# chrischoy/DeepGlobalRegistration

Measured on AMD Instinct MI355X. Metric: pair registrations/sec (FCGF x2 + 1-NN + 6-D inlier net + gate + weighted Procrustes + SE(3) refinement), higher is better.
Workload: dtype f32 results via 2 x f16 split operands (3 f16 MFMA products per MAC, f32 accumulate); k = 1 convs, kNN re-evaluation and registration in exact f32, SVD in f64

## Files before the change

deepglobalregistration_amd/_lib.py:

```python
import ctypes as C
import os
import threading

import torch

_HERE = os.path.dirname(os.path.abspath(__file__))
LIB_PATH = os.environ.get('DGR_HIP_LIB') or os.path.join(_HERE, 'lib', 'libdgr_hip.so')

DGR_OK, DGR_EINVAL, DGR_EHIP, DGR_ENOMEM, DGR_ESVD, DGR_EINTERNAL = 0, -1, -2, -3, -4, -5
STATUS_OK, STATUS_LOW_CONFIDENCE, STATUS_SVD_FAILED, STATUS_SAFEGUARD = 0, 1, 2, 3
STATUS_FLAG_ICP_SKIPPED, STATUS_MASK = 0x100, 0xff

c_i32p, c_i64p, c_f32p, c_f64p = (C.POINTER(C.c_int32), C.POINTER(C.c_int64),
                                  C.POINTER(C.c_float), C.POINTER(C.c_double))
vp = C.c_void_p


class WeightDesc(C.Structure):
    _fields_ = [('name', C.c_char_p), ('data', vp), ('numel', C.c_int64)]


class Params(C.Structure):
    _fields_ = [('clip_weight_thresh', C.c_float), ('voxel_size', C.c_float),
                ('inlier_feature_type', C.c_int), ('max_iter', C.c_int),
                ('max_break_count', C.c_int), ('break_threshold_ratio', C.c_double),
                ('skip_refinement', C.c_int), ('safeguard', C.c_int), ('ransac_hypotheses', C.c_int64),
                ('ransac_seed', C.c_uint32), ('use_icp', C.c_int)]


class PgParams(C.Structure):
    _fields_ = [('mu', C.c_double), ('reference_node', C.c_int), ('max_iter', C.c_int), ('rel_tol', C.c_double)]


SIGNATURES = {
    'dgr_last_error': (C.c_char_p, []),
    'dgr_version': (C.c_char_p, []),
    'dgr_ctx_create': (C.c_int, [C.c_int, C.POINTER(vp)]),
    'dgr_ctx_destroy': (None, [vp]),
    'dgr_ctx_workspace_bytes': (C.c_int64, [vp]),
    'dgr_ctx_create_partition_stream': (C.c_int, [vp, C.c_int, C.c_int, C.POINTER(vp)]),
    'dgr_voxelize': (C.c_int, [vp, vp, C.c_int, C.c_int64, C.c_double, C.c_int32, vp, vp, vp, c_i64p, vp]),
    'dgr_net_create': (C.c_int, [vp, C.c_int, C.c_int, C.c_int, C.c_int, C.c_int,
                                 C.POINTER(WeightDesc), C.c_int, C.POINTER(vp)]),
    'dgr_net_create_device': (C.c_int, [vp, C.c_int, C.c_int, C.c_int, C.c_int, C.c_int,
                                        C.POINTER(WeightDesc), C.c_int, C.POINTER(vp)]),
    'dgr_net_destroy': (None, [vp]),
    'dgr_net_param_bytes': (C.c_int64, [vp]),
    'dgr_net_share': (C.c_int, [vp, vp, C.POINTER(vp)]),
    'dgr_net_sharers': (C.c_int, [vp]),
    'dgr_net_set_wide_coarse': (C.c_int, [vp, C.c_int]),
    'dgr_resunet_forward': (C.c_int, [vp, vp, vp, vp, C.c_int64, vp, vp]),
    'dgr_net_get_intermediate': (C.c_int, [vp, vp, C.c_char_p, vp, C.c_int64, c_i64p, c_i64p]),
    'dgr_net_get_tensor': (C.c_int, [vp, vp, C.c_char_p, C.c_int, vp, C.c_int64, c_i64p, c_i64p]),
    'dgr_net_layer_stats': (C.c_int, [vp, vp, C.c_int, c_i64p]),
    'dgr_net_num_layers': (C.c_int, [vp]),
    'dgr_net_rerun_layer': (C.c_int, [vp, vp, C.c_int, C.c_int, c_f32p, c_f32p]),
    'dgr_maps_create': (C.c_int, [vp, vp, C.c_int64, C.c_int, C.c_int, C.POINTER(vp), vp]),
    'dgr_maps_destroy': (None, [vp]),
    'dgr_maps_get_coords': (C.c_int, [vp, C.c_int, vp, C.c_int64, c_i64p]),
    'dgr_maps_get_kernel_map': (C.c_int, [vp, C.c_int, C.c_int, vp, C.c_int64, vp, vp, C.c_int64,
                                          c_i64p, c_i64p]),
    'dgr_maps_create_ex': (C.c_int, [vp, vp, C.c_int64, C.c_int, C.c_int, C.c_int, C.POINTER(vp), vp]),
    'dgr_maps_get_raw': (C.c_int, [vp, C.c_char_p, C.c_int, C.c_char_p, vp, C.c_int64, c_i64p, c_i64p]),
# ... 142 lines not shown
```

deepglobalregistration_amd/csrc/ctx.hip:

```cpp
#include <stdarg.h>
#include <time.h>
#include <string.h>

#include "dgr_internal.h"

static thread_local char g_err[1024] = "";

void dgr_set_error(const char *fmt, ...) {
  va_list ap;
  va_start(ap, fmt);
  vsnprintf(g_err, sizeof(g_err), fmt, ap);
  va_end(ap);
}

extern "C" const char *dgr_last_error(void) { return g_err; }
extern "C" const char *dgr_version(void) { return "dgr_hip 0.4 (gfx950)"; }

static constexpr size_t kAlign = 256;
static constexpr size_t kMinChunk = (size_t)256 << 20;

bool dgr_workspace_fill(uint32_t *word) {
  static const char *env = getenv("DGR_WORKSPACE_FILL");
  static const uint32_t w = env ? (uint32_t)strtoul(env, nullptr, 16) : 0u;
  if (word) *word = w;
  return env != nullptr;
// ... 89 lines not shown
  }
  return ev[used++];
}

void DgrEventPool::release() {
  for (auto e : ev) (void)hipEventDestroy(e);
  ev.clear();
  used = 0;
}

extern "C" int dgr_ctx_create(int device, dgr_ctx **out) {
  DGR_REQUIRE(out != nullptr, "dgr_ctx_create: out is NULL");
  int count = 0;
  DGR_HIP_CHECK(hipGetDeviceCount(&count));
  DGR_REQUIRE(device >= 0 && device < count, "dgr_ctx_create: device %d out of range (%d visible)",
              device, count);
  DGR_HIP_CHECK(hipSetDevice(device));
  hipDeviceProp_t prop;
  DGR_HIP_CHECK(hipGetDeviceProperties(&prop, device));
  dgr_ctx *ctx = new dgr_ctx();
  ctx->device = device;
  ctx->num_cus = prop.multiProcessorCount > 0 ? prop.multiProcessorCount : 256;
  ctx->all_cus = ctx->num_cus;
  *out = ctx;
  return DGR_OK;
}

extern "C" int dgr_ctx_create_partition_stream(dgr_ctx *ctx, int part, int nparts, dgr_stream *out) {
  DGR_REQUIRE(ctx != nullptr && out != nullptr, "dgr_ctx_create_partition_stream: NULL argument");
  DGR_REQUIRE(nparts == 1 || nparts == 2 || nparts == 4, "partition stream: nparts = %d (1, 2 or 4)", nparts);
  DGR_REQUIRE(part >= 0 && part < nparts, "partition stream: part %d of %d", part, nparts);
  DGR_HIP_CHECK(hipSetDevice(ctx->device));
  *out = nullptr;
  if (ctx->part_stream) {
    DGR_HIP_CHECK(hipDeviceSynchronize());
    DGR_HIP_CHECK(hipStreamDestroy(ctx->part_stream));
    ctx->part_stream = nullptr;
    ctx->num_cus = ctx->all_cus;
  }
  if (nparts == 1) return DGR_OK;
  const int n = ctx->all_cus, xcds = 8;
  DGR_REQUIRE(n % (xcds * 8) == 0, "partition stream: %d compute units are not 8 XCDs x 8 k slots", n);
  const int words = (n + 31) / 32;
  std::vector<uint32_t> mask(words, 0u);
  int mine = 0;
  for (int b = 0; b < n; ++b)
// ... 14 lines not shown
    ctx->pin_bytes = 0;
    const size_t want = bytes < 4096 ? 4096 : bytes * 2;
    DGR_HIP_CHECK(hipHostMalloc((void **)&ctx->pin, want, hipHostMallocDefault));
    ctx->pin_bytes = want;
  }
  *out = ctx->pin;
  return DGR_OK;
}

int dgr_ctx_wait(dgr_ctx *ctx, hipStream_t stream, long predicted_ns) {
  static const bool spin = getenv("DGR_SPIN_SYNC") != nullptr;
  if (spin) {
    DGR_HIP_CHECK(hipStreamSynchronize(stream));
    return DGR_OK;
  }
  if (!ctx->wait_ev) DGR_HIP_CHECK(hipEventCreateWithFlags(&ctx->wait_ev, hipEventDisableTiming));
  DGR_HIP_CHECK(hipEventRecord(ctx->wait_ev, stream));
  struct timespec t0, t1;
  clock_gettime(CLOCK_MONOTONIC, &t0);
  auto elapsed_ns = [&]() -> long {
    clock_gettime(CLOCK_MONOTONIC, &t1);
    return (t1.tv_sec - t0.tv_sec) * 1000000000l + (t1.tv_nsec - t0.tv_nsec);
  };
  if (predicted_ns > 300000) {
    const long ns = predicted_ns / 5 * 4;
    struct timespec first = {ns / 1000000000l, ns % 1000000000l};
    nanosleep(&first, nullptr);
  }
  for (;;) {
    const hipError_t e = hipEventQuery(ctx->wait_ev);
    if (e == hipSuccess) break;
    if (e != hipErrorNotReady) DGR_HIP_CHECK(e);
    const long el = elapsed_ns();
    if (predicted_ns > 300000 && el < predicted_ns + predicted_ns / 10) {
      if (predicted_ns > 8000000) {
        struct timespec nap = {0, 30000};
        nanosleep(&nap, nullptr);
      }
      continue;
    }
    long ns = el / 64;
    struct timespec nap = {0, ns < 10000 ? 10000 : ns > 200000 ? 200000 : ns};
    nanosleep(&nap, nullptr);
  }
  ctx->last_wait_ns = elapsed_ns();
  return DGR_OK;
}

extern "C" void dgr_ctx_destroy(dgr_ctx *ctx) {
  if (!ctx) return;
  (void)hipSetDevice(ctx->device);
  (void)hipDeviceSynchronize();
  if (ctx->wait_ev) (void)hipEventDestroy(ctx->wait_ev);
  if (ctx->pin) (void)hipHostFree(ctx->pin);
  if (ctx->part_stream) (void)hipStreamDestroy(ctx->part_stream);
  ctx->arena.release();
  ctx->events.release();
  delete ctx;
}

extern "C" int64_t dgr_ctx_workspace_bytes(dgr_ctx *ctx) {
  return ctx ? (int64_t)ctx->arena.reserved() : 0;
}

extern "C" int dgr_debug_workspace_peek(dgr_ctx *ctx, int64_t nwords, uint32_t *host_out) {
  DGR_REQUIRE(ctx != nullptr && host_out != nullptr && nwords > 0, "dgr_debug_workspace_peek: bad argument");
  DGR_HIP_CHECK(hipSetDevice(ctx->device));
  DGR_HIP_CHECK(hipDeviceSynchronize());
  DGR_CHECK(ctx->arena.reset());
  uint32_t *p;
  DGR_ALLOC(p, ctx->arena, uint32_t, nwords);
// ... 80 lines not shown
```

deepglobalregistration_amd/csrc/dgr_internal.h:

```cpp
#pragma once
#include <hip/hip_runtime.h>
#include <stdint.h>
#include <stdio.h>
#include <stdlib.h>
#include <string>
#include <vector>

#include "../../include/dgr_hip.h"

void dgr_set_error(const char *fmt, ...);

#define DGR_HIP_CHECK(expr)                                                                  \
  do {                                                                                       \
    hipError_t _e = (expr);                                                                  \
    if (_e != hipSuccess) {                                                                  \
      dgr_set_error("%s:%d: %s failed: %s", __FILE__, __LINE__, #expr, hipGetErrorString(_e)); \
      return DGR_EHIP;                                                                       \
    }                                                                                        \
  } while (0)

#define DGR_CHECK(expr)          \
  do {                           \
    int _r = (expr);             \
    if (_r != DGR_OK) return _r; \
  } while (0)

#define DGR_REQUIRE(cond, ...)     \
  do {                             \
    if (!(cond)) {                 \
// ... 185 lines not shown
int dgr_conv_dense_launch(const DgrConvOsLaunch &a, hipStream_t stream, const char **kernel_name = nullptr);
bool dgr_conv_up_supported(int cin, int cin_pad, int cout);
int dgr_conv_up_launch(const DgrConvOsLaunch &a, hipStream_t stream, const char **kernel_name = nullptr);
int dgr_l2_normalize_rows(const float *in, int in_ld, float *out, int out_ld, int c, int relu,
                          const int32_t *n_dev, int64_t n_cap, hipStream_t stream);

struct DgrBatchOutputs {
  const void *ptr[5] = {nullptr, nullptr, nullptr, nullptr, nullptr};
  int64_t numel[5] = {0, 0, 0, 0, 0};
  uint64_t generation = 0;
};

struct DgrEventPool {
  std::vector<hipEvent_t> ev;
  size_t used = 0;
  hipEvent_t next();
  void release();
};

constexpr int DGR_KNN_TRACE_FIELDS = 8;

struct dgr_ctx {
  int device = 0;
  int num_cus = 256;
  DgrArena arena;
  bool profiling = false;
  float stage_ms[9] = {0, 0, 0, 0, 0, 0, 0, 0, 0};
  int64_t conv_launches = 0;
  DgrBatchOutputs last;
  std::vector<double> last_T64;
  DgrEventPool events;
  std::vector<std::pair<hipEvent_t, hipEvent_t>> conv_spans, gemm_spans, map3_spans, map6_spans;
  std::vector<float> conv_span_ms, gemm_span_ms;
  std::vector<unsigned long long *> conv_clks;
  std::vector<float> conv_clk_us;
  std::vector<const char *> conv_kinds;
  int32_t *flag_dev = nullptr;
  hipEvent_t wait_ev = nullptr;
  long last_wait_ns = 0;
  double batch_ns_per_row = 0;
  double pairs_ns_per_row = 0;
  unsigned char *pin = nullptr;
  size_t pin_bytes = 0;
  hipStream_t part_stream = nullptr;
  int all_cus = 256;
  bool knn_trace = false;
  std::vector<int32_t> knn_trace_rows;
  std::vector<int64_t> knn_trace_q0;
};

int dgr_ctx_pinned(dgr_ctx *ctx, size_t bytes, unsigned char **out);
int dgr_flag_error(int32_t flag);

int dgr_ctx_wait(dgr_ctx *ctx, hipStream_t stream, long predicted_ns = 0);

int dgr_resunet_forward_impl(dgr_ctx *ctx, dgr_net *net, const int32_t *coords, const float *feats,
                             int64_t N, float *out, hipStream_t stream);
int dgr_ctx_collect_profile(dgr_ctx *ctx);
void dgr_ctx_begin_profile(dgr_ctx *ctx);

int dgr_knn1_batch_impl(dgr_ctx *ctx, const float *F0, const int64_t *off0, const float *F1, const int64_t *off1,
                        int npairs, int C, int squared, int64_t *idx_out, float *dist_out, hipStream_t stream);
int dgr_knn1_impl(dgr_ctx *ctx, const float *F0, int64_t N0, const float *F1, int64_t N1, int C,
                  int squared, int64_t *idx_out, float *dist_out, hipStream_t stream);
int dgr_inlier_inputs_impl(const int32_t *coords0, const float *xyz0, int64_t N0,
                           const int32_t *coords1, const float *xyz1, const int64_t *idx1,
                           int feature_type, int32_t *coords6, float *feats, hipStream_t stream);
int dgr_icp_impl(dgr_ctx *ctx, const float *src, int64_t N0, const float *dst, int64_t N1, double max_dist,
                 const double *T_init, int max_iter, double rel_fitness, double rel_rmse, double *T_out,
                 double *stats_out, hipStream_t stream);
int dgr_ransac_impl(dgr_ctx *ctx, const float *X, const float *Y, int64_t N, double max_dist, int64_t num_hypotheses,
                    uint32_t seed, double *T_out, double *stats_out, hipStream_t stream);
// ... 44 lines not shown
```

deepglobalregistration_amd/csrc/net.hip:

```cpp
#include <math.h>
#include <stdlib.h>
#include <string.h>

#include <algorithm>
#include <memory>
#include <string>

#include "dgr_internal.h"

constexpr int CH[5] = {0, 32, 64, 128, 256};
constexpr int TR[5] = {0, 64, 64, 64, 128};
static constexpr float BN_EPS = 1e-5f;

enum Tn : int { NO = -1, X, T1, Y1, CAT1, S1T, S1, T2, Y2, CAT2, S2T, S2, T4, Y4, CAT4, S4T, S4, T8, Y8, S8,
                U4, V4, U2, V2, U1, V1, H, OUT, N_TENSORS };
constexpr int W_CIN = -1, W_COUT = -2;
struct TensorRow { const char *name; int lvl; Tn buf; int col0, cols, relu; };
static const TensorRow TENSORS[N_TENSORS] = {
    {"X", 0, X, 0, W_CIN, 0},
    {"T1", 0, T1, 0, CH[1], 0}, {"Y1", 0, Y1, 0, CH[1], 1},
    {"CAT1", 0, CAT1, 0, TR[2] + CH[1], 1}, {"S1T", 0, CAT1, 0, TR[2], 1}, {"S1", 0, CAT1, TR[2], CH[1], 1},
    {"T2", 1, T2, 0, CH[2], 0}, {"Y2", 1, Y2, 0, CH[2], 1},
    {"CAT2", 1, CAT2, 0, TR[3] + CH[2], 1}, {"S2T", 1, CAT2, 0, TR[3], 1}, {"S2", 1, CAT2, TR[3], CH[2], 1},
    {"T4", 2, T4, 0, CH[3], 0}, {"Y4", 2, Y4, 0, CH[3], 1},
// ... 737 lines not shown
      const LayerRow &row = LAYERS[li];
      const DgrLayer &L = net->W->layers[li];
      maps[li] = map_of(ms, row.map, TENSORS[row.in].lvl, TENSORS[row.out].lvl);
      kinds[li] = layer_kind(ms, f.wide3, L, maps[li], row.res != NO, ms.cm[TENSORS[row.in].lvl].n_cap,
                             net->width(TENSORS[row.in].buf));
      if (rule_major(kinds[li])) need = std::max(need, maps[li].km->pair_cap * L.cout);
    }
    DGR_ALLOC(f.ybuf, A, float, need);
  }
  Tensor t[N_TENSORS];
  const bool fuse_l2 = net->normalize && net->cout <= 32;
  for (int i = 0; i < N_TENSORS; ++i) {
    const TensorRow &row = TENSORS[i];
    t[i].ld = net->width(row.buf);
    t[i].relu = row.relu;
    if (row.buf != i) t[i].ptr = t[row.buf].ptr + row.col0;
    else if (i == X) t[i].ptr = const_cast<float *>(feats);
    else if (i == OUT && (!net->normalize || fuse_l2)) t[i].ptr = out;
    else t[i].ptr = A.get<float>((size_t)ms.cm[row.lvl].n_cap * t[i].ld);
    if (!t[i].ptr) return DGR_ENOMEM;
  }
  DGR_CHECK(derive_forms(f, kinds, t));

  for (int li = 0; li < N_LAYERS; ++li) {
    const LayerRow &row = LAYERS[li];
    DGR_CHECK(f.conv(li, kinds[li], t[row.in], maps[li], TENSORS[row.in].lvl, TENSORS[row.out].lvl, t[row.out],
                     row.res != NO ? &t[row.res] : nullptr, fuse_l2 && row.out == OUT));
  }
  if (t[OUT].ptr != out) {
    DGR_CHECK(dgr_l2_normalize_rows(t[OUT].ptr, net->cout, out, net->cout, net->cout, 0, ms.cm[0].n_dev, ms.cm[0].n_cap, stream));
    t[OUT].ptr = out;
  }

  net->run_generation = ctx->arena.generation;
  std::copy(t, t + N_TENSORS, net->tensors);
  std::copy(ms.cm, ms.cm + 4, net->levels);
  return DGR_OK;
}

void dgr_ctx_begin_profile(dgr_ctx *ctx) {
  ctx->events.used = 0;
  ctx->conv_spans.clear();
  ctx->gemm_spans.clear();
  ctx->conv_kinds.clear();
  ctx->conv_clks.clear();
  ctx->map3_spans.clear();
  ctx->map6_spans.clear();
  ctx->conv_launches = 0;
}

// ... 266 lines not shown
```

deepglobalregistration_amd/csrc/pipeline.hip:

```cpp
#include <string.h>

#include "dgr_internal.h"

__global__ void inlier_inputs_kernel(const int32_t *__restrict__ coords0, const float *__restrict__ xyz0,
                                     int64_t N0, const int32_t *__restrict__ coords1,
                                     const float *__restrict__ xyz1, const int64_t *__restrict__ idx1,
                                     int feature_type, int32_t *__restrict__ coords6,
                                     float *__restrict__ feats) {
  const int64_t i = (int64_t)blockIdx.x * blockDim.x + threadIdx.x;
  if (i >= N0) return;
  const int64_t j = idx1[i];
#pragma unroll
  for (int d = 0; d < 4; ++d) coords6[i * 7 + d] = coords0[i * 4 + d];
#pragma unroll
  for (int d = 0; d < 3; ++d) coords6[i * 7 + 4 + d] = coords1[j * 4 + 1 + d];
  if (feature_type == 0) {
    feats[i] = 1.f;
  } else {
#pragma unroll
    for (int d = 0; d < 3; ++d) {
      feats[i * 6 + d] = cosf(xyz0[i * 3 + d]);
      feats[i * 6 + 3 + d] = cosf(xyz1[j * 3 + d]);
    }
  }
// ... 111 lines not shown
  int64_t *idx1, *off0_dev;
  int32_t *coords6;
  float *feats6, *logit, *weights;
  DgrRegResult *res_dev;
};

static int alloc_batch_buffers(DgrArena &A, int64_t n0, int npairs, const int64_t *off0, hipStream_t stream,
                               BatchBuffers *B) {
  DGR_ALLOC(B->idx1, A, int64_t, n0);
  DGR_ALLOC(B->coords6, A, int32_t, n0 * 7);
  DGR_ALLOC(B->feats6, A, float, n0 * 6);
  DGR_ALLOC(B->logit, A, float, n0);
  DGR_ALLOC(B->weights, A, float, n0);
  DGR_ALLOC(B->off0_dev, A, int64_t, npairs + 1);
  DGR_ALLOC(B->res_dev, A, DgrRegResult, npairs);
  DGR_HIP_CHECK(hipMemcpyAsync(B->off0_dev, off0, (size_t)(npairs + 1) * sizeof(int64_t), hipMemcpyHostToDevice, stream));
  return DGR_OK;
}

static int register_from_features(dgr_ctx *ctx, dgr_net *inlier, const int32_t *coords0, const float *xyz0,
                                  const int64_t *off0, const int32_t *coords1, const float *xyz1, const int64_t *off1,
                                  const float *F0, const float *F1, int C, int npairs, const dgr_params *prm,
                                  const int64_t *override_idx1, const float *forced_logit, const BatchBuffers &B,
                                  StageTimer &tm, double *ns_per_row, float *T_out, int32_t *status_out,
                                  float *stats_out, hipStream_t stream);

extern "C" int dgr_register_batch(dgr_ctx *ctx, dgr_net *fcgf, dgr_net *inlier, const int32_t *coords0,
                                  const float *xyz0, const int64_t *off0, const int32_t *coords1,
                                  const float *xyz1, const int64_t *off1, int npairs, const dgr_params *prm,
                                  const int64_t *override_idx1, const float *forced_logit, float *T_out,
                                  int32_t *status_out,
                                  float *stats_out, dgr_stream stream_) {
  DGR_REQUIRE(ctx && fcgf && inlier && coords0 && xyz0 && off0 && coords1 && xyz1 && off1 && prm && T_out &&
                  status_out,
              "dgr_register_batch: NULL argument");
  DGR_REQUIRE(npairs >= 1 && npairs <= 65535, "dgr_register_batch: npairs=%d out of range", npairs);
  DGR_REQUIRE(dgr_net_dim(fcgf) == 3 && dgr_net_dim(inlier) == 6 && dgr_net_in_channels(fcgf) == 1,
              "dgr_register_batch: expects the 3-D FCGF net (1 input channel) and the 6-D inlier net");
  const int ftype = prm->inlier_feature_type;
  DGR_REQUIRE((ftype == 0 && dgr_net_in_channels(inlier) == 1) || (ftype == 1 && dgr_net_in_channels(inlier) == 6),
              "inlier_feature_type %d does not match the inlier network input width %d", ftype,
              dgr_net_in_channels(inlier));
  for (int p = 0; p < npairs; ++p)
    DGR_REQUIRE(off0[p + 1] > off0[p] && off1[p + 1] > off1[p], "pair %d is empty", p);
  DGR_REQUIRE(dgr_net_ctx(fcgf) == ctx && dgr_net_ctx(inlier) == ctx,
              "dgr_register_batch: a net object belongs to another context (one dgr_net per context: dgr_net_share)");
  hipStream_t stream = (hipStream_t)stream_;
// ... 7 lines not shown
  const int C = dgr_net_out_channels(fcgf);
  StageTimer tm{ctx, stream, {}, ctx->profiling};

  float *F0, *F1, *ones;
  BatchBuffers B;
  DGR_ALLOC(F0, A, float, (n0 + n1) * C);
  F1 = F0 + n0 * C;
  DGR_ALLOC(ones, A, float, n0 + n1);
  DGR_CHECK(alloc_batch_buffers(A, n0, npairs, off0, stream, &B));
  fill_kernel<<<256, 256, 0, stream>>>(ones, n0 + n1, 1.f);

  DGR_CHECK(tm.rec(0, 0));
  {
    DgrArena::Mark mk = A.mark();
    int32_t *coords01;
    DGR_ALLOC(coords01, A, int32_t, (n0 + n1) * 4);
    concat_coords_kernel<<<(int)dgr_ceil_div(n0 + n1, 256), 256, 0, stream>>>(coords0, n0, coords1, n1, coords01);
    DGR_CHECK(dgr_resunet_forward_impl(ctx, fcgf, coords01, ones, n0 + n1, F0, stream));
    A.rewind(mk);
    dgr_net_invalidate_runs(fcgf);
  }
  DGR_CHECK(tm.rec(0, 1));
  return register_from_features(ctx, inlier, coords0, xyz0, off0, coords1, xyz1, off1, F0, F1, C, npairs, prm,
                                override_idx1, forced_logit, B, tm, &ctx->batch_ns_per_row, T_out, status_out, stats_out,
                                stream);
}

static int register_from_features(dgr_ctx *ctx, dgr_net *inlier, const int32_t *coords0, const float *xyz0,
                                  const int64_t *off0, const int32_t *coords1, const float *xyz1, const int64_t *off1,
                                  const float *F0, const float *F1, int C, int npairs, const dgr_params *prm,
                                  const int64_t *override_idx1, const float *forced_logit, const BatchBuffers &B,
                                  StageTimer &tm, double *ns_per_row, float *T_out, int32_t *status_out,
                                  float *stats_out, hipStream_t stream) {
  DgrArena &A = ctx->arena;
  const int64_t n0 = off0[npairs], n1 = off1[npairs];
  const int ftype = prm->inlier_feature_type;
  int64_t *const idx1 = B.idx1, *const off0_dev = B.off0_dev;
  int32_t *const coords6 = B.coords6;
  float *const feats6 = B.feats6, *const logit = B.logit, *const weights = B.weights;
  DgrRegResult *const res_dev = B.res_dev;
  DGR_CHECK(tm.rec(1, 0));
  DGR_CHECK(dgr_knn1_batch_impl(ctx, F0, off0, F1, off1, npairs, C, 0, idx1, nullptr, stream));
  if (override_idx1)
    override_idx_kernel<<<(int)dgr_ceil_div(n0, 256), 256, 0, stream>>>(idx1, override_idx1, n0);
  DGR_CHECK(tm.rec(1, 1));
  DGR_CHECK(tm.rec(2, 0));
  DGR_CHECK(dgr_inlier_inputs_impl(coords0, xyz0, n0, coords1, xyz1, idx1, ftype, coords6, feats6, stream));
  DGR_CHECK(tm.rec(2, 1));
  DGR_CHECK(tm.rec(3, 0));
  {
    DgrArena::Mark mk = A.mark();
    DGR_CHECK(dgr_resunet_forward_impl(ctx, inlier, coords6, feats6, n0, logit, stream));
    A.rewind(mk);
    dgr_net_invalidate_runs(inlier);
  }
  DGR_CHECK(tm.rec(3, 1));
  DGR_CHECK(tm.rec(4, 0));
  const float eps = 1.1920928955078125e-07f;
  DGR_CHECK(dgr_registration_launch_ctx(ctx, xyz0, xyz1, idx1, forced_logit ? forced_logit : logit, 1,
                                        prm->clip_weight_thresh, off0_dev, off0, npairs, n0, 2.f * prm->voxel_size,
                                        prm->max_iter, prm->max_break_count, prm->break_threshold_ratio,
                                        prm->skip_refinement, 1, eps, weights, res_dev, stream));
  DGR_CHECK(tm.rec(4, 1));

  unsigned char *pin;
  DGR_CHECK(dgr_ctx_pinned(ctx, 64 + (size_t)npairs * sizeof(DgrRegResult), &pin));
  const DgrRegResult *res = reinterpret_cast<const DgrRegResult *>(pin + 64);
  DGR_HIP_CHECK(hipMemcpyAsync(pin + 64, res_dev, (size_t)npairs * sizeof(DgrRegResult), hipMemcpyDeviceToHost, stream));
  DGR_HIP_CHECK(hipMemcpyAsync(pin, ctx->flag_dev, sizeof(int32_t), hipMemcpyDeviceToHost, stream));
  DGR_CHECK(dgr_ctx_wait(ctx, stream, (long)(*ns_per_row * (double)(n0 + n1))));
  *ns_per_row = (double)ctx->last_wait_ns / (double)(n0 + n1);
  DGR_CHECK(dgr_flag_error(*reinterpret_cast<volatile int32_t *>(pin)));
  for (int p = 0; p < npairs; ++p)
    if (res[p].status == DGR_STATUS_EXCHANGE_TIMEOUT) {
      dgr_set_error("registration of pair %d: the workgroups sharing the pair lost each other (exchange timed out)", p);
      return DGR_EINTERNAL;
    }
  for (int p = 0; p < npairs; ++p) {
    float *T = T_out + p * 16;
    const DgrRegResult &r = res[p];
    for (int i = 0; i < 16; ++i) T[i] = (i % 5 == 0) ? 1.f : 0.f;
    if (r.status == DGR_STATUS_OK) {
      for (int i = 0; i < 3; ++i) {
        for (int j = 0; j < 3; ++j) T[i * 4 + j] = r.R[i * 3 + j];
        T[i * 4 + 3] = r.t[i];
      }
    }
    status_out[p] = r.status;
    if (stats_out) {
      stats_out[p * 4 + 0] = (float)r.iterations;
      stats_out[p * 4 + 1] = r.loss;
      stats_out[p * 4 + 2] = (float)r.break_count;
      stats_out[p * 4 + 3] = r.wsum;
    }
// ... 173 lines not shown
  DGR_CHECK(dgr_ctx_new_flag(ctx, stream));
  DgrArena &A = ctx->arena;
  StageTimer tm{ctx, stream, {}, ctx->profiling};

  int32_t *coords;
  float *xyz, *F0;
  BankSegment *segs_dev;
  BatchBuffers B;
  DGR_ALLOC(F0, A, float, (n0 + n1) * C);
  DGR_ALLOC(coords, A, int32_t, (n0 + n1) * 4);
  DGR_ALLOC(xyz, A, float, (n0 + n1) * 3);
  DGR_ALLOC(segs_dev, A, BankSegment, segs.size());
  auto run = [&]() -> int {
    DGR_CHECK(alloc_batch_buffers(A, n0, npairs, off0.data(), stream, &B));
    DGR_CHECK(tm.rec(0, 0));
    DGR_HIP_CHECK(hipMemcpyAsync(segs_dev, segs.data(), segs.size() * sizeof(BankSegment), hipMemcpyHostToDevice, stream));
    bank_gather_kernel<<<(int)dgr_ceil_div(n0 + n1, BANK_GATHER_ROWS), BANK_GATHER_ROWS, 0, stream>>>(
        reinterpret_cast<const int4 *>(bank_coords), bank_xyz, reinterpret_cast<const float4 *>(bank_F), segs_dev,
        2 * npairs, n0 + n1, C == 16 ? 2 : C == 32 ? 3 : 4, reinterpret_cast<int4 *>(coords), xyz,
        reinterpret_cast<float4 *>(F0));
    DGR_LAUNCH_CHECK();
    DGR_CHECK(tm.rec(0, 1));
    return register_from_features(ctx, inlier, coords, xyz, off0.data(), coords + n0 * 4, xyz + n0 * 3, off1.data(), F0,
                                  F0 + n0 * C, C, npairs, prm, override_idx1, forced_logit, B, tm, &ctx->pairs_ns_per_row,
                                  T_out, status_out, stats_out, stream);
  };
  const int rc = run();
  if (rc != DGR_OK) (void)hipStreamSynchronize(stream);
  return rc;
}

extern "C" int dgr_register_batch_f64(dgr_ctx *ctx, double *T_out, int64_t capacity_pairs, int64_t *npairs) {
  DGR_REQUIRE(ctx && npairs, "dgr_register_batch_f64: NULL argument");
  const int64_t n = (int64_t)(ctx->last_T64.size() / 16);
  DGR_REQUIRE(n > 0, "no dgr_register_batch has run on this ctx");
  *npairs = n;
  if (T_out) {
    DGR_REQUIRE(capacity_pairs >= n, "destination buffer too small");
    memcpy(T_out, ctx->last_T64.data(), (size_t)n * 16 * sizeof(double));
  }
  return DGR_OK;
}

extern "C" int dgr_register_batch_output(dgr_ctx *ctx, int which, void *dst_dev, int64_t capacity_bytes,
                                         int64_t *numel, dgr_stream stream) {
  DGR_REQUIRE(ctx && numel && which >= 0 && which < 5, "dgr_register_batch_output: bad argument");
  DGR_REQUIRE(ctx->last.ptr[which] != nullptr, "no dgr_register_batch has run on this ctx");
// ... 13 lines not shown
```

deepglobalregistration_amd/ops.py:

```python
import ctypes as C

import numpy as np
import torch

from . import _args, _lib
from ._lib import check, get_ctx, ptr, stream_ptr, vp

F32_EPS = float(np.finfo(np.float32).eps)

_NP_PTR = {np.dtype(np.int32): _lib.c_i32p, np.dtype(np.int64): _lib.c_i64p, np.dtype(np.float32): _lib.c_f32p,
           np.dtype(np.float64): _lib.c_f64p, np.dtype(np.uint8): C.POINTER(C.c_uint8)}


def _np_ptr(a):
    return None if a is None else a.ctypes.data_as(_NP_PTR[a.dtype])


def _dev(t):
    if not (torch.is_tensor(t) and t.is_cuda):
        raise ValueError('expected a CUDA(ROCm) tensor')
    return t.device


def _as(t, dtype, device):
# ... 912 lines not shown
_BATCH_OUT = {'idx1': (0, torch.int64), 'logit': (1, torch.float32), 'weights': (2, torch.float32),
              'F0': (3, torch.float32), 'F1': (4, torch.float32)}


def batch_output(device, which):
    lib = _lib.load()
    dev = torch.device(device)
    wid, dtype = _BATCH_OUT[which]
    n = C.c_int64(0)
    check(lib.dgr_register_batch_output(get_ctx(dev), wid, None, 0, C.byref(n), stream_ptr(dev.index)))
    out = torch.empty(n.value, dtype=dtype, device=dev)
    check(lib.dgr_register_batch_output(get_ctx(dev), wid, ptr(out), out.numel() * out.element_size(),
                                        C.byref(n), stream_ptr(dev.index)))
    return out


def partition_stream(device, part, nparts):
    device = torch.device(device)
    h = vp()
    check(_lib.load().dgr_ctx_create_partition_stream(get_ctx(device), int(part), int(nparts), C.byref(h)))
    return torch.cuda.ExternalStream(h.value, device) if h.value else None


def set_profiling(device, enable):
    check(_lib.load().dgr_ctx_set_profiling(get_ctx(device), int(bool(enable))))


def stage_times(device):
    t = (C.c_float * 16)()
    n = C.c_int(0)
    check(_lib.load().dgr_ctx_stage_times_v2(get_ctx(device), t, 16, C.byref(n)))
    names = ['fcgf', 'knn', 'inlier_inputs', 'inlier_net', 'registration', 'maps_3d', 'maps_6d', 'conv_kernels', 'o3d_steps']
    out = dict(zip(names, [float(v) for v in t[:n.value]]))
    out['conv_launches'] = int(_lib.load().dgr_ctx_conv_launches(get_ctx(device)))
    return out


def conv_launch_times(device):
    cap = 4096
    t, g = (C.c_float * cap)(), (C.c_float * cap)()
    n = C.c_int64(0)
    check(_lib.load().dgr_ctx_conv_launch_times(get_ctx(device), t, g, cap, C.byref(n)))
    return [float(t[i]) for i in range(n.value)], [float(g[i]) for i in range(n.value)]


def conv_launch_kernel_us(device):
# ... 37 lines not shown
```

include/dgr_hip.h:

```cpp
#ifndef DGR_HIP_H
#define DGR_HIP_H

#include <stdint.h>

#ifdef __cplusplus
extern "C" {
#endif

typedef struct dgr_ctx dgr_ctx;
typedef struct dgr_net dgr_net;
typedef struct dgr_maps dgr_maps;
typedef void *dgr_stream;

enum {
  DGR_OK = 0,
  DGR_EINVAL = -1,
  DGR_EHIP = -2,
  DGR_ENOMEM = -3,
  DGR_ESVD = -4,
  DGR_EINTERNAL = -5
};

enum { DGR_STATUS_OK = 0, DGR_STATUS_LOW_CONFIDENCE = 1, DGR_STATUS_SVD_FAILED = 2,
       DGR_STATUS_SAFEGUARD = 3 ,
       DGR_STATUS_FLAG_ICP_SKIPPED = 0x100, DGR_STATUS_MASK = 0xff,
       DGR_STATUS_EXCHANGE_TIMEOUT = 0x7f };

const char *dgr_last_error(void);
const char *dgr_version(void);

int dgr_ctx_create(int device, dgr_ctx **out);
void dgr_ctx_destroy(dgr_ctx *ctx);
int64_t dgr_ctx_workspace_bytes(dgr_ctx *ctx);
int dgr_ctx_create_partition_stream(dgr_ctx *ctx, int part, int nparts, dgr_stream *out);

int dgr_voxelize(dgr_ctx *ctx, const void *xyz, int is_f64, int64_t M, double voxel_size,
                 int32_t batch_index, int64_t *sel_out, int32_t *coords_out, float *xyz_out,
                 int64_t *n_out, dgr_stream stream);

typedef struct {
  const char *name;
  const float *data;
  int64_t numel;
} dgr_weight_desc;

int dgr_net_create(dgr_ctx *ctx, int D, int in_channels, int out_channels, int conv1_kernel_size,
                   int normalize_feature, const dgr_weight_desc *weights, int n_weights,
                   dgr_net **out);
int dgr_net_create_device(dgr_ctx *ctx, int D, int in_channels, int out_channels, int conv1_kernel_size,
                          int normalize_feature, const dgr_weight_desc *weights, int n_weights,
                          dgr_net **out);
void dgr_net_destroy(dgr_net *net);
int64_t dgr_net_param_bytes(const dgr_net *net);
int dgr_net_share(dgr_ctx *ctx, const dgr_net *src, dgr_net **out);
int dgr_net_sharers(const dgr_net *net);
int dgr_net_set_wide_coarse(dgr_net *net, int on);

// ... 175 lines not shown
```

Before: 407.6.

## Add cross-partition heavy-layer gate and robust wait-time predictor

Adds a per-device ticket gate that limits how many partition streams can run the two wide 256-channel 6-D conv layers at once, using HIP events so one partition waits for an earlier one. The goal is less contention when partitions overlap their heaviest layers, at the cost of added cross-stream dependencies and host-side mutex/condvar waits. The gate defaults to width 0, so it is off. Separately, the host wait predictor is replaced with a learner that uses only polled observations and halves its estimate after an oversleep, to avoid sleeping past kernel completion.

```diff
diff --git a/deepglobalregistration_amd/_lib.py b/deepglobalregistration_amd/_lib.py
--- a/deepglobalregistration_amd/_lib.py
+++ b/deepglobalregistration_amd/_lib.py
@@ -39,6 +39,9 @@
     'dgr_ctx_destroy': (None, [vp]),
     'dgr_ctx_workspace_bytes': (C.c_int64, [vp]),
     'dgr_ctx_create_partition_stream': (C.c_int, [vp, C.c_int, C.c_int, C.POINTER(vp)]),
+    'dgr_heavy_gate_configure': (C.c_int, [C.c_int, C.c_int, C.c_int64]),
+    'dgr_heavy_gate_set_trace': (C.c_int, [C.c_int, C.c_int]),
+    'dgr_heavy_gate_get_trace': (C.c_int, [C.c_int, C.c_int64, c_i32p, c_f32p, c_f32p, c_i64p, c_i64p, c_i64p]),
     'dgr_voxelize': (C.c_int, [vp, vp, C.c_int, C.c_int64, C.c_double, C.c_int32, vp, vp, vp, c_i64p, vp]),
     'dgr_net_create': (C.c_int, [vp, C.c_int, C.c_int, C.c_int, C.c_int, C.c_int,
                                  C.POINTER(WeightDesc), C.c_int, C.POINTER(vp)]),
diff --git a/deepglobalregistration_amd/csrc/ctx.hip b/deepglobalregistration_amd/csrc/ctx.hip
--- a/deepglobalregistration_amd/csrc/ctx.hip
+++ b/deepglobalregistration_amd/csrc/ctx.hip
@@ -1,6 +1,8 @@
 #include <stdarg.h>
 #include <time.h>
 #include <string.h>
+
+#include <atomic>
 
 #include "dgr_internal.h"
 
@@ -136,6 +138,8 @@
   ctx->device = device;
   ctx->num_cus = prop.multiProcessorCount > 0 ? prop.multiProcessorCount : 256;
   ctx->all_cus = ctx->num_cus;
+  static std::atomic<int> next_id{0};
+  ctx->id = next_id++;
   *out = ctx;
   return DGR_OK;
 }
@@ -196,15 +200,17 @@
     clock_gettime(CLOCK_MONOTONIC, &t1);
     return (t1.tv_sec - t0.tv_sec) * 1000000000l + (t1.tv_nsec - t0.tv_nsec);
   };
-  if (predicted_ns > 300000) {
-    const long ns = predicted_ns / 5 * 4;
-    struct timespec first = {ns / 1000000000l, ns % 1000000000l};
+  const long first_ns = wait_first_sleep_ns(predicted_ns);
+  if (first_ns > 0) {
+    struct timespec first = {first_ns / 1000000000l, first_ns % 1000000000l};
     nanosleep(&first, nullptr);
   }
+  ctx->last_wait_polled = first_ns == 0;
   for (;;) {
     const hipError_t e = hipEventQuery(ctx->wait_ev);
     if (e == hipSuccess) break;
     if (e != hipErrorNotReady) DGR_HIP_CHECK(e);
+    ctx->last_wait_polled = true;
     const long el = elapsed_ns();
     if (predicted_ns > 300000 && el < predicted_ns + predicted_ns / 10) {
       if (predicted_ns > 8000000) {
@@ -221,6 +227,118 @@
   return DGR_OK;
 }
 
+static constexpr int kGateDevices = 64, kGateTraceCap = 4096;
+static thread_local int g_gate_ctx_id = -1;
+
+int DgrGateEvents::record(int slot, hipStream_t s) {
+  if (!ev[slot]) DGR_HIP_CHECK(hipEventCreateWithFlags(&ev[slot], hipEventDisableTiming));
+  DGR_HIP_CHECK(hipEventRecord(ev[slot], s));
+  return DGR_OK;
+}
+
+int DgrGateEvents::wait(int slot, hipStream_t s) {
+  if (ev[slot]) DGR_HIP_CHECK(hipStreamWaitEvent(s, ev[slot], 0));
+  return DGR_OK;
+}
+
+int DgrGateEvents::trace(long ticket, int end, hipStream_t s) {
+  std::lock_guard<std::mutex> g(mu);
+  const long i = ticket - base;
+  if (i < 0 || i >= kGateTraceCap) return DGR_OK;
+  if ((long)marks.size() <= i) marks.resize((size_t)i + 1);
+  Mark &m = marks[i];
+  if (!m.e[end]) DGR_HIP_CHECK(hipEventCreate(&m.e[end]));
+  DGR_HIP_CHECK(hipEventRecord(m.e[end], s));
+  m.set[end] = true;
+  if (!end) m.ctx_id = g_gate_ctx_id;
+  return DGR_OK;
+}
+
+struct DeviceGate {
+  DgrGateEvents events;
+  DgrHeavyGate gate;
+  DeviceGate(int width, long min_rows) : gate(&events, width, min_rows) {}
+};
+
+static int gate_default_width() {
+  static const char *env = getenv("DGR_HEAVY_GATE");
+  static const int w = env ? DgrHeavyGate::clamp(atoi(env)) : DGR_HEAVY_GATE_WIDTH;
+  return w;
+}
+
+static DeviceGate *device_gate(int device) {
+  static std::mutex mu;
+  static DeviceGate *gates[kGateDevices] = {};
+  if (device < 0 || device >= kGateDevices) return nullptr;
+  std::lock_guard<std::mutex> g(mu);
+  if (!gates[device]) gates[device] = new DeviceGate(gate_default_width(), DGR_HEAVY_GATE_MIN_ROWS);
+  return gates[device];
+}
+
+DgrHeavyGate *dgr_heavy_gate_for(dgr_ctx *ctx, int64_t rows, hipStream_t stream) {
+  if (!ctx->part_stream || stream != ctx->part_stream) return nullptr;
+  DeviceGate *d = device_gate(ctx->device);
+  if (!d || !d->gate.applies((long)rows)) return nullptr;
+  g_gate_ctx_id = ctx->id;
+  return &d->gate;
+}
+
+static int gate_device(const char *who, int device, DeviceGate **out) {
+  int count = 0;
+  DGR_HIP_CHECK(hipGetDeviceCount(&count));
+  DGR_REQUIRE(device >= 0 && device < count && device < kGateDevices, "%s: device %d out of range (%d visible)", who, device, count);
+  *out = device_gate(device);
+  return DGR_OK;
+}
+
+extern "C" int dgr_heavy_gate_configure(int device, int width, int64_t min_rows) {
+  DGR_REQUIRE(width >= 0 && width <= 64, "dgr_heavy_gate_configure: width %d (0 = off, at most 64)", width);
+  DGR_REQUIRE(min_rows >= 0, "dgr_heavy_gate_configure: min_rows %lld is negative", (long long)min_rows);
+  DeviceGate *d;
+  DGR_CHECK(gate_device("dgr_heavy_gate_configure", device, &d));
+  d->gate.configure(width, (long)min_rows);
+  return DGR_OK;
+}
+
+extern "C" int dgr_heavy_gate_set_trace(int device, int enable) {
+  DeviceGate *d;
+  DGR_CHECK(gate_device("dgr_heavy_gate_set_trace", device, &d));
+  DGR_HIP_CHECK(hipSetDevice(device));
+  DGR_HIP_CHECK(hipDeviceSynchronize());
+  d->gate.set_trace(enable != 0);
+  long base = 0;
+  d->gate.counters(&base, nullptr, nullptr);
+  std::lock_guard<std::mutex> g(d->events.mu);
+  d->events.base = base;
+  for (auto &m : d->events.marks) { m.set[0] = m.set[1] = false; m.ctx_id = -1; }
+  return DGR_OK;
+}
+
+extern "C" int dgr_heavy_gate_get_trace(int device, int64_t capacity, int32_t *ctx_ids, float *start_ms, float *end_ms,
+                                        int64_t *n, int64_t *tickets, int64_t *waits) {
+  DGR_REQUIRE(n != nullptr && capacity >= 0 && (capacity == 0 || (ctx_ids && start_ms && end_ms)),
+              "dgr_heavy_gate_get_trace: bad argument");
+  DeviceGate *d;
+  DGR_CHECK(gate_device("dgr_heavy_gate_get_trace", device, &d));
+  DGR_HIP_CHECK(hipSetDevice(device));
+  DGR_HIP_CHECK(hipDeviceSynchronize());
+  long issued = 0, nwaits = 0;
+  d->gate.counters(nullptr, &issued, &nwaits);
+  if (tickets) *tickets = issued;
+  if (waits) *waits = nwaits;
+  std::lock_guard<std::mutex> g(d->events.mu);
+  const auto &marks = d->events.marks;
+  int64_t m = 0;
+  while (m < (int64_t)marks.size() && marks[m].set[0] && marks[m].set[1]) ++m;
+  *n = m;
+  for (int64_t i = 0; i < m && i < capacity; ++i) {
+    ctx_ids[i] = marks[i].ctx_id;
+    DGR_HIP_CHECK(hipEventElapsedTime(&start_ms[i], marks[0].e[0], marks[i].e[0]));
+    DGR_HIP_CHECK(hipEventElapsedTime(&end_ms[i], marks[0].e[0], marks[i].e[1]));
+  }
+  return DGR_OK;
+}
+
 extern "C" void dgr_ctx_destroy(dgr_ctx *ctx) {
   if (!ctx) return;
   (void)hipSetDevice(ctx->device);
diff --git a/deepglobalregistration_amd/csrc/dgr_internal.h b/deepglobalregistration_amd/csrc/dgr_internal.h
--- a/deepglobalregistration_amd/csrc/dgr_internal.h
+++ b/deepglobalregistration_amd/csrc/dgr_internal.h
@@ -3,8 +3,12 @@
 #include <stdint.h>
 #include <stdio.h>
 #include <stdlib.h>
+#include <mutex>
 #include <string>
 #include <vector>
+
+#include "heavy_gate.h"
+#include "wait_predictor.h"
 
 #include "../../include/dgr_hip.h"
 
@@ -236,6 +240,7 @@
 
 struct dgr_ctx {
   int device = 0;
+  int id = 0;
   int num_cus = 256;
   DgrArena arena;
   bool profiling = false;
@@ -252,8 +257,9 @@
   int32_t *flag_dev = nullptr;
   hipEvent_t wait_ev = nullptr;
   long last_wait_ns = 0;
-  double batch_ns_per_row = 0;
-  double pairs_ns_per_row = 0;
+  bool last_wait_polled = true;
+  WaitPredictor batch_wait;
+  WaitPredictor pairs_wait;
   unsigned char *pin = nullptr;
   size_t pin_bytes = 0;
   hipStream_t part_stream = nullptr;
@@ -262,6 +268,20 @@
   std::vector<int32_t> knn_trace_rows;
   std::vector<int64_t> knn_trace_q0;
 };
+
+struct DgrGateEvents {
+  int record(int slot, hipStream_t s);
+  int wait(int slot, hipStream_t s);
+  int trace(long ticket, int end, hipStream_t s);
+  hipEvent_t ev[64] = {};
+  struct Mark { int ctx_id = -1; hipEvent_t e[2] = {nullptr, nullptr}; bool set[2] = {false, false}; };
+  std::mutex mu;
+  std::vector<Mark> marks;
+  long base = 0;
+};
+using DgrHeavyGate = HeavyGate<DgrGateEvents, hipStream_t, 64>;
+using DgrHeavyScope = HeavyGateScope<DgrHeavyGate, hipStream_t>;
+DgrHeavyGate *dgr_heavy_gate_for(dgr_ctx *ctx, int64_t rows, hipStream_t stream);
 
 int dgr_ctx_pinned(dgr_ctx *ctx, size_t bytes, unsigned char **out);
 int dgr_flag_error(int32_t flag);
diff --git a/deepglobalregistration_amd/csrc/heavy_gate.h b/deepglobalregistration_amd/csrc/heavy_gate.h
--- /dev/null
+++ b/deepglobalregistration_amd/csrc/heavy_gate.h
@@ -0,0 +1,113 @@
+#pragma once
+#include <condition_variable>
+#include <mutex>
+
+template <class B, class Stream, int RING = 64>
+class HeavyGate {
+  static_assert(RING >= 2, "a ring of at least two slots");
+
+ public:
+  explicit HeavyGate(B *backend, int width = 0, long min_rows = 0) : b_(backend), width_(clamp(width)), min_rows_(min_rows) {
+    for (int i = 0; i < RING; ++i) left_[i] = entered_[i] = -1;
+  }
+  HeavyGate(const HeavyGate &) = delete;
+  HeavyGate &operator=(const HeavyGate &) = delete;
+
+  static int clamp(int w) { return w < 0 ? 0 : w > RING ? RING : w; }
+  void configure(int width, long min_rows) {
+    std::lock_guard<std::mutex> g(mu_);
+    width_ = clamp(width);
+    min_rows_ = min_rows;
+  }
+  int width() const { std::lock_guard<std::mutex> g(mu_); return width_; }
+  long min_rows() const { std::lock_guard<std::mutex> g(mu_); return min_rows_; }
+  bool applies(long rows) const { std::lock_guard<std::mutex> g(mu_); return width_ > 0 && rows >= min_rows_; }
+
+  void set_trace(bool on) {
+    std::lock_guard<std::mutex> g(mu_);
+    trace_ = on;
+    trace_base_ = next_;
+    issued_ = waits_ = 0;
+  }
+  void counters(long *base, long *issued, long *waits) const {
+    std::lock_guard<std::mutex> g(mu_);
+    if (base) *base = trace_base_;
+    if (issued) *issued = issued_;
+    if (waits) *waits = waits_;
+  }
+
+  int enter(Stream s, long *ticket) {
+    std::unique_lock<std::mutex> lk(mu_);
+    *ticket = -1;
+    const int W = width_;
+    if (W == 0) return 0;
+    const long t = next_++;
+    *ticket = t;
+    ++issued_;
+    const bool tr = trace_;
+    int rc = 0;
+    if (t >= W) {
+      const long dep = t - W, old = t - RING + W;
+      cv_.wait(lk, [&] { return left_[dep % RING] >= dep && (old < 0 || old >= t || entered_[old % RING] >= old); });
+      ++waits_;
+      lk.unlock();
+      rc = b_->wait((int)(dep % RING), s);
+      lk.lock();
+    }
+    entered_[t % RING] = t;
+    lk.unlock();
+    cv_.notify_all();
+    if (rc == 0 && tr) rc = b_->trace(t, 0, s);
+    return rc;
+  }
+
+  int leave(long ticket, Stream s) {
+    if (ticket < 0) return 0;
+    bool tr;
+    { std::lock_guard<std::mutex> g(mu_); tr = trace_ && ticket >= trace_base_; }
+    int rc = tr ? b_->trace(ticket, 1, s) : 0;
+    const int rc2 = b_->record((int)(ticket % RING), s);
+    {
+      std::lock_guard<std::mutex> g(mu_);
+      left_[ticket % RING] = ticket;
+    }
+    cv_.notify_all();
+    return rc ? rc : rc2;
+  }
+
+ private:
+  B *b_;
+  mutable std::mutex mu_;
+  std::condition_variable cv_;
+  int width_;
+  long min_rows_;
+  long next_ = 0;
+  long left_[RING], entered_[RING];
+  bool trace_ = false;
+  long trace_base_ = 0, issued_ = 0, waits_ = 0;
+};
+
+template <class G, class Stream>
+class HeavyGateScope {
+ public:
+  HeavyGateScope() = default;
+  HeavyGateScope(const HeavyGateScope &) = delete;
+  HeavyGateScope &operator=(const HeavyGateScope &) = delete;
+  ~HeavyGateScope() { (void)leave(); }
+  int enter(G *gate, Stream s) {
+    gate_ = gate;
+    s_ = s;
+    return gate->enter(s, &ticket_);
+  }
+  int leave() {
+    const long t = ticket_;
+    ticket_ = -1;
+    return t >= 0 ? gate_->leave(t, s_) : 0;
+  }
+  long ticket() const { return ticket_; }
+
+ private:
+  G *gate_ = nullptr;
+  Stream s_{};
+  long ticket_ = -1;
+};
diff --git a/deepglobalregistration_amd/csrc/net.hip b/deepglobalregistration_amd/csrc/net.hip
--- a/deepglobalregistration_amd/csrc/net.hip
+++ b/deepglobalregistration_amd/csrc/net.hip
@@ -783,10 +783,24 @@
   }
   DGR_CHECK(derive_forms(f, kinds, t));
 
+  int heavy0 = -1, heavy1 = -1;
+  for (int li = 0; li < N_LAYERS; ++li) {
+    if (LAYERS[li].in == T8 && LAYERS[li].out == Y8) heavy0 = li;
+    if (LAYERS[li].in == Y8 && LAYERS[li].out == S8) heavy1 = li;
+  }
+  auto wide256 = [&](int li) {
+    const DgrLayer &L = net->W->layers[li];
+    return kinds[li] == K_WIDE && L.cin_pad == 256 && L.cout_pad == 256;
+  };
+  DgrHeavyGate *const gate = net->D == 6 && heavy0 >= 0 && heavy1 > heavy0 && wide256(heavy0) && wide256(heavy1)
+                                 ? dgr_heavy_gate_for(ctx, ms.cm[TENSORS[T8].lvl].n_cap, stream) : nullptr;
+  DgrHeavyScope heavy;
   for (int li = 0; li < N_LAYERS; ++li) {
     const LayerRow &row = LAYERS[li];
+    if (gate && li == heavy0) DGR_CHECK(heavy.enter(gate, stream));
     DGR_CHECK(f.conv(li, kinds[li], t[row.in], maps[li], TENSORS[row.in].lvl, TENSORS[row.out].lvl, t[row.out],
                      row.res != NO ? &t[row.res] : nullptr, fuse_l2 && row.out == OUT));
+    if (gate && li == heavy1) DGR_CHECK(heavy.leave());
   }
   if (t[OUT].ptr != out) {
     DGR_CHECK(dgr_l2_normalize_rows(t[OUT].ptr, net->cout, out, net->cout, net->cout, 0, ms.cm[0].n_dev, ms.cm[0].n_cap, stream));
diff --git a/deepglobalregistration_amd/csrc/pipeline.hip b/deepglobalregistration_amd/csrc/pipeline.hip
--- a/deepglobalregistration_amd/csrc/pipeline.hip
+++ b/deepglobalregistration_amd/csrc/pipeline.hip
@@ -157,7 +157,7 @@
                                   const int64_t *off0, const int32_t *coords1, const float *xyz1, const int64_t *off1,
                                   const float *F0, const float *F1, int C, int npairs, const dgr_params *prm,
                                   const int64_t *override_idx1, const float *forced_logit, const BatchBuffers &B,
-                                  StageTimer &tm, double *ns_per_row, float *T_out, int32_t *status_out,
+                                  StageTimer &tm, WaitPredictor *wait, float *T_out, int32_t *status_out,
                                   float *stats_out, hipStream_t stream);
 
 extern "C" int dgr_register_batch(dgr_ctx *ctx, dgr_net *fcgf, dgr_net *inlier, const int32_t *coords0,
@@ -211,7 +211,7 @@
   }
   DGR_CHECK(tm.rec(0, 1));
   return register_from_features(ctx, inlier, coords0, xyz0, off0, coords1, xyz1, off1, F0, F1, C, npairs, prm,
-                                override_idx1, forced_logit, B, tm, &ctx->batch_ns_per_row, T_out, status_out, stats_out,
+                                override_idx1, forced_logit, B, tm, &ctx->batch_wait, T_out, status_out, stats_out,
                                 stream);
 }
 
@@ -219,7 +219,7 @@
                                   const int64_t *off0, const int32_t *coords1, const float *xyz1, const int64_t *off1,
                                   const float *F0, const float *F1, int C, int npairs, const dgr_params *prm,
                                   const int64_t *override_idx1, const float *forced_logit, const BatchBuffers &B,
-                                  StageTimer &tm, double *ns_per_row, float *T_out, int32_t *status_out,
+                                  StageTimer &tm, WaitPredictor *wait, float *T_out, int32_t *status_out,
                                   float *stats_out, hipStream_t stream) {
   DgrArena &A = ctx->arena;
   const int64_t n0 = off0[npairs], n1 = off1[npairs];
@@ -257,8 +257,8 @@
   const DgrRegResult *res = reinterpret_cast<const DgrRegResult *>(pin + 64);
   DGR_HIP_CHECK(hipMemcpyAsync(pin + 64, res_dev, (size_t)npairs * sizeof(DgrRegResult), hipMemcpyDeviceToHost, stream));
   DGR_HIP_CHECK(hipMemcpyAsync(pin, ctx->flag_dev, sizeof(int32_t), hipMemcpyDeviceToHost, stream));
-  DGR_CHECK(dgr_ctx_wait(ctx, stream, (long)(*ns_per_row * (double)(n0 + n1))));
-  *ns_per_row = (double)ctx->last_wait_ns / (double)(n0 + n1);
+  DGR_CHECK(dgr_ctx_wait(ctx, stream, wait->predict((long)(n0 + n1))));
+  wait->learn((long)(n0 + n1), ctx->last_wait_ns, ctx->last_wait_polled);
   DGR_CHECK(dgr_flag_error(*reinterpret_cast<volatile int32_t *>(pin)));
   for (int p = 0; p < npairs; ++p)
     if (res[p].status == DGR_STATUS_EXCHANGE_TIMEOUT) {
@@ -478,7 +478,7 @@
     DGR_LAUNCH_CHECK();
     DGR_CHECK(tm.rec(0, 1));
     return register_from_features(ctx, inlier, coords, xyz, off0.data(), coords + n0 * 4, xyz + n0 * 3, off1.data(), F0,
-                                  F0 + n0 * C, C, npairs, prm, override_idx1, forced_logit, B, tm, &ctx->pairs_ns_per_row,
+                                  F0 + n0 * C, C, npairs, prm, override_idx1, forced_logit, B, tm, &ctx->pairs_wait,
                                   T_out, status_out, stats_out, stream);
   };
   const int rc = run();
diff --git a/deepglobalregistration_amd/csrc/wait_predictor.h b/deepglobalregistration_amd/csrc/wait_predictor.h
--- /dev/null
+++ b/deepglobalregistration_amd/csrc/wait_predictor.h
@@ -0,0 +1,25 @@
+#pragma once
+
+struct WaitPredictor {
+  double ns_per_row = 0;
+  double obs[2] = {0, 0};
+  int n_obs = 0;
+
+  long predict(long rows) const { return (long)(ns_per_row * (double)rows); }
+
+  void learn(long rows, long elapsed_ns, bool polled) {
+    if (rows <= 0) return;
+    const double per_row = (double)elapsed_ns / (double)rows;
+    if (polled) {
+      obs[1] = obs[0];
+      obs[0] = per_row;
+      if (n_obs < 2) ++n_obs;
+      ns_per_row = n_obs == 2 && obs[1] < obs[0] ? obs[1] : obs[0];
+    } else {
+      ns_per_row = 0.5 * (per_row < ns_per_row ? per_row : ns_per_row);
+      n_obs = 0;
+    }
+  }
+};
+
+inline long wait_first_sleep_ns(long predicted_ns) { return predicted_ns > 300000 ? predicted_ns / 5 * 4 : 0; }
diff --git a/deepglobalregistration_amd/ops.py b/deepglobalregistration_amd/ops.py
--- a/deepglobalregistration_amd/ops.py
+++ b/deepglobalregistration_amd/ops.py
@@ -958,6 +958,45 @@
     return torch.cuda.ExternalStream(h.value, device) if h.value else None
 
 
+def check_heavy_gate_args(device, width=None, min_rows=None):
+    device = torch.device(device)
+    if device.type != 'cuda':
+        raise ValueError(f'the heavy gate belongs to a GPU, got device {device}')
+    index = 0 if device.index is None else device.index
+    if device.index is None and torch.cuda.is_available():
+        index = torch.cuda.current_device()
+    index = _args.integer(index, 'device index', lambda v: 0 <= v < max(1, torch.cuda.device_count()),
+                          'the index of a visible GPU')
+    if width is not None:
+        width = _args.integer(width, 'width', lambda v: 0 <= v <= 64, 'an integer from 0 (off) to 64')
+    if min_rows is not None:
+        min_rows = _args.integer(min_rows, 'min_rows', lambda v: 0 <= v < 2 ** 63, 'an integer >= 0')
+    return index, width, min_rows
+
+
+def heavy_gate_configure(device, width=0, min_rows=32768):
+    index, width, min_rows = check_heavy_gate_args(device, width, min_rows)
+    check(_lib.load().dgr_heavy_gate_configure(index, width, min_rows))
+
+
+def heavy_gate_trace(device, enable):
+    index, _, _ = check_heavy_gate_args(device)
+    check(_lib.load().dgr_heavy_gate_set_trace(index, int(bool(enable))))
+
+
+def heavy_gate_trace_rows(device):
+    index, _, _ = check_heavy_gate_args(device)
+    lib = _lib.load()
+    n, tickets, waits = C.c_int64(0), C.c_int64(0), C.c_int64(0)
+    check(lib.dgr_heavy_gate_get_trace(index, 0, None, None, None, C.byref(n), C.byref(tickets), C.byref(waits)))
+    cap = max(1, n.value)
+    ids, t0, t1 = np.zeros(cap, np.int32), np.zeros(cap, np.float32), np.zeros(cap, np.float32)
+    check(lib.dgr_heavy_gate_get_trace(index, cap, ids.ctypes.data_as(_lib.c_i32p), t0.ctypes.data_as(_lib.c_f32p),
+                                       t1.ctypes.data_as(_lib.c_f32p), C.byref(n), C.byref(tickets), C.byref(waits)))
+    m = min(n.value, cap)
+    return ids[:m], np.stack([t0[:m], t1[:m]], 1), tickets.value, waits.value
+
+
 def set_profiling(device, enable):
     check(_lib.load().dgr_ctx_set_profiling(get_ctx(device), int(bool(enable))))
 
diff --git a/include/dgr_hip.h b/include/dgr_hip.h
--- a/include/dgr_hip.h
+++ b/include/dgr_hip.h
@@ -33,6 +33,12 @@
 void dgr_ctx_destroy(dgr_ctx *ctx);
 int64_t dgr_ctx_workspace_bytes(dgr_ctx *ctx);
 int dgr_ctx_create_partition_stream(dgr_ctx *ctx, int part, int nparts, dgr_stream *out);
+#define DGR_HEAVY_GATE_WIDTH 0
+#define DGR_HEAVY_GATE_MIN_ROWS 32768
+int dgr_heavy_gate_configure(int device, int width, int64_t min_rows);
+int dgr_heavy_gate_set_trace(int device, int enable);
+int dgr_heavy_gate_get_trace(int device, int64_t capacity, int32_t *ctx_ids, float *start_ms, float *end_ms, int64_t *n,
+                             int64_t *tickets, int64_t *waits);
 
 int dgr_voxelize(dgr_ctx *ctx, const void *xyz, int is_f64, int64_t M, double voxel_size,
                  int32_t batch_index, int64_t *sel_out, int32_t *coords_out, float *xyz_out,
```

Result: no change. 408.1, median of 2 (+0.1%).
